# Ophiase/Stochastic-Vector-Oracle-Consensus

Hardware: AMD Instinct MI355X
Metric: consensus updates/sec (N oracles x D dims, batched) (higher is better)
Workload: dtype fp32; 1 GPU; model=svoc-consensus N=256 D=4096 streaming (f=32, constrained), global_batch=1024, seq_len=4096, parallelism=dp1, engine_mode=fast, storage=fp32, n_oracles=256, dimension=4096, n_failing=32, hip_graph=True, backend_world=1, stream_pool=89, independent_failing=False, transactional=False, fast_transactional=True, pipeline_chunks=2

## Files before the change

csrc/bindings/torch_ops.cpp:

```cpp
#include <cstdlib>
#include <ATen/ATen.h>
#include <c10/hip/HIPStream.h>
#include <torch/library.h>

#include <thread>

#include "../engine/engine.hpp"
#include "svoc/route.hpp"
#include "svoc/ops.hpp"

namespace svoc {
namespace {

int cpu_threads() {
  static int n = [] {
    unsigned h = std::thread::hardware_concurrency();
    return (int)(h == 0 ? 1 : (h > 32 ? 32 : h));
  }();
  return n;
}

void check_out(const at::Tensor& t, at::ScalarType dt, std::initializer_list<int64_t> shape, const char* name,
               const at::Device& dev) {
  TORCH_CHECK(t.scalar_type() == dt, name, ": wrong dtype ", t.scalar_type());
// ... 26 lines not shown
  check_out(qr, at::kFloat, {B, N}, "qr", dev);
  check_out(reliable, at::kByte, {B, N}, "reliable", dev);
  check_out(status, at::kInt, {B}, "status", dev);
}

void fast_round_cpu(const at::Tensor& values, const c10::optional<at::Tensor>& active, int64_t D,
                    int64_t n_failing, bool constrained, double max_spread, at::Tensor c1, at::Tensor cons,
                    at::Tensor skew, at::Tensor kurt, at::Tensor rel, at::Tensor qr, at::Tensor reliable,
                    at::Tensor status, int64_t wave_hint, int64_t mode, int64_t rel_dim, bool legacy,
                    const c10::optional<at::Tensor>& work, const c10::optional<at::Tensor>& stats,
                    const c10::optional<at::Tensor>& upd_rows, const c10::optional<at::Tensor>& upd_oracle,
                    const c10::optional<at::Tensor>& upd_status, int64_t upd_per_inst,
                    const c10::optional<at::Tensor>& rst_saved, const c10::optional<at::Tensor>& rst_saved_en,
                    const c10::optional<at::Tensor>& rst_enabled, const c10::optional<at::Tensor>& rst_n_active,
                    const c10::optional<at::Tensor>& pend_rows, const c10::optional<at::Tensor>& pend_oracle,
                    const c10::optional<at::Tensor>& pend_status) {
  (void)wave_hint;
  (void)work;
  (void)stats;
  TORCH_CHECK(!upd_rows.has_value() || !upd_rows->defined(), "fused transactional streaming is a GPU path");
  TORCH_CHECK(!rst_saved.has_value() || !rst_saved->defined(), "in-kernel rollback is a GPU path");
  TORCH_CHECK(!pend_rows.has_value() || !pend_rows->defined(), "the deferred commit is a GPU path");
  (void)pend_oracle;
  (void)pend_status;
  (void)rst_saved_en;
  (void)rst_enabled;
  (void)rst_n_active;
  (void)upd_oracle;
  (void)upd_status;
  (void)upd_per_inst;
  fast_round_checks(values, D, c1, cons, skew, kurt, rel, qr, reliable, status);
  const int64_t B = values.size(0), N = values.size(1), ld = values.size(2), is = values.stride(0);
// ... 33 lines not shown
  fb.rel_dim = rel_dim;
  fb.legacy = legacy;
  fast_round_batch_cpu(fb, cpu_threads());
}

void fast_round_hip(const at::Tensor& values, const c10::optional<at::Tensor>& active, int64_t D,
                    int64_t n_failing, bool constrained, double max_spread, at::Tensor c1, at::Tensor cons,
                    at::Tensor skew, at::Tensor kurt, at::Tensor rel, at::Tensor qr, at::Tensor reliable,
                    at::Tensor status, int64_t wave_hint, int64_t mode, int64_t rel_dim, bool legacy,
                    const c10::optional<at::Tensor>& work, const c10::optional<at::Tensor>& stats,
                    const c10::optional<at::Tensor>& upd_rows, const c10::optional<at::Tensor>& upd_oracle,
                    const c10::optional<at::Tensor>& upd_status, int64_t upd_per_inst,
                    const c10::optional<at::Tensor>& rst_saved, const c10::optional<at::Tensor>& rst_saved_en,
                    const c10::optional<at::Tensor>& rst_enabled, const c10::optional<at::Tensor>& rst_n_active,
                    const c10::optional<at::Tensor>& pend_rows, const c10::optional<at::Tensor>& pend_oracle,
                    const c10::optional<at::Tensor>& pend_status) {
  fast_round_checks(values, D, c1, cons, skew, kurt, rel, qr, reliable, status);
  TORCH_CHECK(values.scalar_type() == at::kBFloat16 || values.scalar_type() == at::kFloat,
              "GPU fast path stores values in bf16 or fp32");
  const bool f32 = values.scalar_type() == at::kFloat;
  const int64_t B = values.size(0), N = values.size(1), ld = values.size(2);
  if (f32) {
    TORCH_CHECK(N >= 2 && N <= 4096, "GPU fp32 fast path supports 2 <= N <= 4096 oracles");
    TORCH_CHECK(B < (1ll << 31) && D < (1 << 30), "size limits");
    TORCH_CHECK(N * ld * 4 < (1ll << 31) && fast_work_words(D) * 4 < (1ll << 31),
                "instance too large for 32-bit buffer offsets (N * ld * 4 B and the workspace must stay < 2 GiB)");
  }
  if (!f32) {
    TORCH_CHECK(N >= 2 && N <= 4096, "GPU fast path supports 2 <= N <= 4096 oracles");
    TORCH_CHECK(ld % 8 == 0, "row stride (ld) must be a multiple of 8 bf16 (16 B)");
    TORCH_CHECK(((uintptr_t)values.data_ptr() & 15) == 0 && values.stride(0) % 8 == 0, "values must be 16-B aligned");
// ... 40 lines not shown
    p.work = (uint32_t*)wtmp.data_ptr();
    p.work_fresh = 1;
  }
  {
    const char* wc = std::getenv("SVOC_WIN_CANCEL");
    p.win_cancel = wc ? (float)std::atof(wc) : 64.f;
  }
  p.work_pairs = (int)fast_work_pairs(D);
  p.work_stride = words;
  auto stream = c10::hip::getCurrentHIPStream(values.device().index()).stream();
  p.c1_out = mode == 0 ? c1.data_ptr<float>() : nullptr;
  if (stats.has_value() && stats->defined()) {
    TORCH_CHECK(stats->scalar_type() == at::kInt && stats->numel() >= 1 && stats->device() == values.device(),
                "stats: int32 [>= 1] on the values' device ([0] += pruned-network fallbacks)");
    p.net_fallbacks = (unsigned int*)stats->data_ptr();
  }
  for (const c10::optional<at::Tensor>* t : {&upd_rows, &upd_oracle, &upd_status, &rst_saved, &rst_saved_en,
                                              &rst_enabled, &rst_n_active})
    TORCH_CHECK(!t->has_value() || !(*t)->defined() || (*t)->device() == values.device(),
                "fast_round: every update / rollback tensor must be on the values' device");
  if (upd_rows.has_value() && upd_rows->defined()) {
    TORCH_CHECK(upd_per_inst <= route.fused_max_u, "fused streaming: this round's kernel takes at most ",
                route.fused_max_u, " updates per instance (fp32 storage, whole constrained rounds on the window "
                "kernel; svoc.ops.fast_route)");
    TORCH_CHECK(upd_per_inst > 0 && upd_oracle.has_value() && upd_status.has_value(), "fused streaming: "
                "upd_oracle, upd_status and upd_per_inst > 0 go with upd_rows");
    const int64_t n = B * upd_per_inst;
    TORCH_CHECK(upd_rows->scalar_type() == values.scalar_type() && upd_rows->is_contiguous() && upd_rows->dim() == 2 &&
                    upd_rows->size(0) == n && upd_rows->size(1) == D && upd_rows->device() == values.device(),
                "upd_rows: contiguous [B * U, D] in the values' dtype on the values' device");
// ... 293 lines not shown
  const int rc = svoc_exact_verdict(&p, stream);
  TORCH_CHECK(rc == 0, "svoc_exact_verdict launch failed: ", rc);
}

}
}

TORCH_LIBRARY(svoc, m) {
  m.def(
      "fast_round(Tensor values, Tensor? active, int D, int n_failing, bool constrained, float max_spread, "
      "Tensor(a!) c1, Tensor(b!) consensus, Tensor(c!) skew, Tensor(d!) kurt, Tensor(e!) rel, Tensor(f!) qr, "
      "Tensor(g!) reliable, Tensor(h!) status, int wave_hint=0, int mode=0, int rel_dim=0, bool legacy=False, "
      "Tensor? work=None, Tensor(i!)? stats=None, Tensor? upd_rows=None, Tensor? upd_oracle=None, "
      "Tensor(j!)? upd_status=None, int upd_per_inst=0, Tensor? rst_saved=None, Tensor? rst_saved_en=None, "
      "Tensor(k!)? rst_enabled=None, Tensor(l!)? rst_n_active=None, Tensor? pend_rows=None, "
      "Tensor? pend_oracle=None, Tensor? pend_status=None) -> ()");
  m.def(
      "exact_round(Tensor values, Tensor? active, int n_failing, bool constrained, int max_spread, "
      "Tensor(a!) c1, Tensor(b!) consensus, Tensor(c!) skew, Tensor(d!) kurt, Tensor(e!) rel, Tensor(f!) qr, "
      "Tensor(g!) reliable, Tensor(h!) status, bool legacy=False, int mode=0, int rel_dim=0, "
      "Tensor(i!)? stats=None) -> ()");
  m.def(
      "exact_verdict(Tensor values, Tensor? active, int n_failing, bool constrained, int max_spread, "
      "Tensor(a!) rel, Tensor(b!) status, bool legacy, Tensor(c!)? stats=None, Tensor(d!)? vstats=None) -> ()");
  m.def("fast_route(int storage, int N, int D, int ld, int n_failing, bool constrained, bool legacy, int mode, "
        "int wave_hint, int work) -> int[]", &svoc::fast_route_op);
  m.def("exact_route(int N, int D, int elem_bytes, int n_failing, bool constrained, bool legacy, int mode) -> int[]",
        &svoc::exact_route_op);
  m.def("fast_work_words(int D) -> int", [](int64_t D) { return svoc::fast_work_words(D); });
  m.def("fast_win_h(int N, int n_failing) -> int",
        [](int64_t N, int64_t f) { return (int64_t)svoc::fast_win_h((int)N, (int)f); });
  svoc::register_extra_defs(m);
}

TORCH_LIBRARY_IMPL(svoc, CPU, m) {
  m.impl("fast_round", &svoc::fast_round_cpu);
  m.impl("exact_round", &svoc::exact_round_cpu);
  m.impl("exact_verdict", &svoc::exact_verdict_cpu);
  svoc::register_extra_cpu(m);
}

TORCH_LIBRARY_IMPL(svoc, CUDA, m) {
  m.impl("fast_round", &svoc::fast_round_hip);
  m.impl("exact_round", &svoc::exact_round_hip);
  m.impl("exact_verdict", &svoc::exact_verdict_hip);
  svoc::register_extra_hip(m);
// ... 2 lines not shown
```

csrc/include/svoc/launch.hpp:

```cpp
#pragma once

#include <stdint.h>

namespace svoc {

struct FastParams {
  const void* values;
  const uint8_t* active;
  int64_t inst_stride;
  int B, N, D, ld;
  int n_failing;
  int constrained;
  float max_spread;
  int wave_hint;
  int mode;
  int rel_dim;
  float* c1;
  float* consensus;
  float* skew;
  float* kurt;
  float* rel;
  float* qr;
  uint8_t* reliable;
  int32_t* status;
// ... 7 lines not shown
  unsigned int* net_fallbacks;
  const float* upd_rows;
  const int64_t* upd_oracle;
  int32_t* upd_status;
  int upd_per_inst;
  const float* pend_rows;
  const int64_t* pend_oracle;
  const int32_t* pend_status;
  const void* rst_saved;
  const uint8_t* rst_saved_en;
  const int64_t* rst_oracle;
  int32_t* rst_status;
  uint8_t* rst_enabled;
  int32_t* rst_n_active;
  int rst_U;
};

inline int64_t fast_work_pairs(int64_t D) { return ((D + 1) / 2 + 255) / 256 * 256; }
inline int64_t fast_work_stage_word(int64_t D) { return fast_work_pairs(D) * (2 * 17 + 8 + 2); }
constexpr int kWinfStageCols = 2 * 17 + 4 + 1;
inline int64_t fast_work_words(int64_t D) { return fast_work_pairs(D) * 2 * (kWinfStageCols + 3); }
inline int64_t fast_work_numel(int64_t B, int64_t D) { return B * fast_work_words(D); }

inline int fast_win_h(int N, int f) {
  const int R = N - f, a = N / 2 - R / 2;
  if (a + 1 <= 5 && f - a + 1 <= 5) return 5;
  if (a + 1 <= 17 && f - a + 1 <= 17) return 17;
  return 0;
}

struct LestParams {
// ... 104 lines not shown
```

csrc/kernels/consensus_fast_winf.hip:

```cpp
#include <hip/hip_runtime.h>
#include <stdint.h>

#include <type_traits>
#include <utility>

#include "svoc/bufload.hpp"
#include "svoc/route.hpp"
#include "svoc/slabdma.hpp"
#include "svoc/rankmask.hpp"
#include "svoc/sortnet.hpp"
#include "svoc/status.hpp"
#include "svoc/verdict.hpp"

namespace svoc {

template <bool CONS>
SVOC_DEV uint32_t fkey(uint32_t raw) {
  if constexpr (CONS) return raw ^ 0x80000000u;
  else return f32_key(raw);
}
template <bool CONS>
SVOC_DEV float fkey_val(uint32_t k) {
  if constexpr (CONS) return __builtin_bit_cast(float, k ^ 0x80000000u);
  else return key_f32(k);
// ... 85 lines not shown
SVOC_DEV bool try_pruned(uint32_t (&r)[64], int seg, int lane, uint32_t (&w)[WN], uint32_t& lo, uint32_t& hi,
                         uint32_t& e0, uint32_t& e63) {
  if constexpr (WN == H && H == 17) {
    bool ok;
    sort_oem<64>(r);
    e0 = r[0];
    e63 = r[63];
    window_group_pruned_sorted<P, H>(r, seg, lane, w, lo, hi, ok);
    return ok;
  } else {
    return false;
  }
}


template <int NSEG, int WAVES, int H, bool CONS, int MODE, bool FUSED = false, bool DEFER = false, bool WIDE = false>
__global__ __launch_bounds__(WAVES * 64) __attribute__((amdgpu_waves_per_eu(2))) void consensus_fast_winf_kernel(FastParams p) {
#pragma clang fp contract(off)
  constexpr int P = 64 / NSEG;
  constexpr int NPAD = 64 * NSEG;
  constexpr int W = WAVES * P;
  constexpr int NT = WAVES * 64;
  constexpr int KEEP = 64 / P;
  constexpr bool PASS1 = MODE != 2;
  __shared__ __attribute__((aligned(16))) uint32_t slab[PASS1 ? WAVES * 64 * 64 : 1];
  __shared__ __attribute__((aligned(16))) float qr_part[WAVES * NPAD];
  __shared__ float qr_lds[NPAD];
  __shared__ uint64_t relmask[4];
  __shared__ int urow[32];
  __shared__ float misc_f[2];
  __shared__ int misc_i[3];
  __shared__ uint32_t redo[128];
  __shared__ int smap[FUSED ? NPAD : 1];
  __shared__ int spend[DEFER ? NPAD : 1];
  __shared__ uint32_t badu[8];

  const int b = blockIdx.x;
  static_assert(!FUSED || (MODE == 0 && CONS), "fused streaming: whole constrained rounds");
  static_assert(!DEFER || FUSED, "deferred commit: a mode of the fused path");
  static_assert(!WIDE || (FUSED && !DEFER), "9-bit piece map: the fused path at 256 updates per instance");
  constexpr bool fused = FUSED;
  const int U = fused ? p.upd_per_inst : 0;
  if (p.active && !p.active[b]) {
    for (int t = threadIdx.x; t < U; t += WAVES * 64) p.upd_status[(int64_t)b * U + t] = ST_NOT_ACTIVE;
    return;
  }
  const int tid = threadIdx.x, lane = tid & 63, wave = __builtin_amdgcn_readfirstlane(tid >> 6);
  if (tid < 32) urow[tid] = 0;
  if (tid == 0) misc_i[2] = 0;
  if (tid < 128) redo[tid] = 0u;
  const int seg = lane / P, cw = lane % P;
  const int N = p.N, D = p.D;
  const int rowb = p.ld * 4;
  const float* inst = (const float*)p.values + (int64_t)b * p.inst_stride;
  const __amdgpu_buffer_rsrc_t rs = instance_rsrc(inst, (uint32_t)(N * rowb));
  const BufDesc rsd = buf_desc(inst, (uint32_t)(N * rowb));
  const int nslab = (D + W - 1) / W;
  const int Dc = 2 * p.work_pairs;
  const __amdgpu_buffer_rsrc_t ws = instance_rsrc(p.work + (int64_t)b * p.work_stride, (uint32_t)(p.work_stride * 4));
  const int MOM = 2 * H * Dc * 4;
  const int LST = MOM + 4 * Dc * 4;
  const int STG = Dc * kWinfStageCols * 4;
  const float* urows = fused ? p.upd_rows + (int64_t)b * U * D : inst;
  const uint32_t ubytes = fused ? (uint32_t)(U * D * 4) : 0u;
  const __amdgpu_buffer_rsrc_t rb = instance_rsrc(urows, ubytes);
// ... 118 lines not shown
            rsd, rbd, reg_o, rowb_o, s * W + wave * P,
            [&](int k) { return ((pm[k / 4] >> (8 * (k % 4))) & 0xffu) | (((ph >> k) & 1u) << 8); },
            [&](int, uint32_t fb) { return (int)__umul24(fb, (unsigned)d4) + cbm; });
      } else
      dma.issue_mapped(
          rsd, rbd, reg_o, rowb_o, s * W + wave * P,
          [&](int k) { return (pm[k / 4] >> (8 * (k % 4))) & 0xffu; },
          [&](int, uint32_t fb) { return (int)__umul24(fb, (unsigned)d4) + cbm; });
    } else {
      dma.issue(rsd, region, rowb, s * W + wave * P);
    }
  };
  for (int attempt = 0; attempt < 2; ++attempt) {
  if (fused) map_pieces();
  if (pass1_slabs > 0) issue_slab(0);
  auto slab_body = [&](auto full_c, int s) __attribute__((always_inline)) {
    constexpr bool FULL = decltype(full_c)::value;
    const int col = s * W + wave * P + cw;
    const bool vc = FULL || col < D;
    int nvl = nv, nll = nl;
    asm volatile("" : "+v"(nvl), "+v"(nll));
    float c1v;
    const uint32_t mW = vc ? 0xffffffffu : 0u;
    RawRows xs;
    __builtin_amdgcn_s_waitcnt(0x0F70);
    if constexpr (DEFER) {
      if (attempt == 0) {
        uint32_t pm[4] = {pmap[0], pmap[1], pmap[2], pmap[3]};
        asm volatile("" : "+v"(pm[0]), "+v"(pm[1]), "+v"(pm[2]), "+v"(pm[3]));
        int rowb_o = rowb;
        asm volatile("" : "+s"(rowb_o));
        const int c0 = s * W + wave * P;
// ... 80 lines not shown
            window_group<NSEG, P, H>(r, seg, lane, wk, klo, khi);
          }
        };
        pruned_net(full_c);
        if constexpr (NSEG == 1) {
#pragma unroll
          for (int m = 0; m < H; ++m) {
            bstore(ws, wk[m], col * 4, 2 * m * Dc * 4);
            bstore(ws, wk[H + m], (Dc + col) * 4, 2 * m * Dc * 4);
          }
        } else {
          constexpr int slo = NSEG == 2 ? 0 : 1;
          if (seg == slo || seg == slo + 1) {
            const int part = seg - slo;
#pragma unroll
            for (int m = 0; m < H; ++m) bstore(ws, wk[m], (part * Dc + col) * 4, 2 * m * Dc * 4);
          }
        }
      } else {
        median_group<NSEG>(r, klo, khi);
      }
      c1v = 0.5f * (fkey_val<CONS>(klo) + fkey_val<CONS>(khi));
    }
    if (seg == 0 && vc) p.c1[(int64_t)b * D + col] = c1v;
    const float cq = vc ? c1v : 0.f;
    f32x2 s1 = {0.f, 0.f}, s2 = s1, s3 = s1, s4 = s1;
    if constexpr (ACC64) {
      qr_moments_regs<!FULL, !FULL>(xs, nvl, cq, mW, acc, s1, s2, s3, s4);
    } else {
      f32x2 slab_acc[32];
#pragma unroll
// ... 5 lines not shown
    if constexpr (NSEG == 4) {
      t1 += xor_lane<16>(t1); t2 += xor_lane<16>(t2); t3 += xor_lane<16>(t3); t4 += xor_lane<16>(t4);
    }
    if constexpr (NSEG >= 2) {
      t1 += xor_lane<32>(t1); t2 += xor_lane<32>(t2); t3 += xor_lane<32>(t3); t4 += xor_lane<32>(t4);
    }
    if (seg == 0) {
      bstore(ws, f2u(t1), col * 4, MOM);
      bstore(ws, f2u(t2), col * 4, MOM + Dc * 4);
      bstore(ws, f2u(t3), col * 4, MOM + 2 * Dc * 4);
      bstore(ws, f2u(t4), col * 4, MOM + 3 * Dc * 4);
    }
  };
  if constexpr (PASS1) {
    const int nfull = N == NPAD ? min(D / W, pass1_slabs) : 0;
#pragma nounroll
    for (int s = 0; s < nfull; ++s) slab_body(std::true_type{}, s);
#pragma nounroll
    for (int s = nfull; s < pass1_slabs; ++s) slab_body(std::false_type{}, s);
  }
  if (!fused) break;
  __syncthreads();
  uint32_t anybad = 0u;
#pragma unroll
  for (int w = 0; w < 8; ++w) anybad |= badu[w];
  if (anybad == 0u || attempt == 1) break;
  if constexpr (FUSED) {
    for (int t = tid; t < NPAD; t += NT)
      if (smap[t] >= 0 && bad_slot(smap[t])) smap[t] = -1;
  }
  __syncthreads();
#pragma unroll
  for (int i = 0; i < (ACC64 ? 32 : 1); ++i) acc[i] = f32x2{0.f, 0.f};
#pragma unroll
// ... 49 lines not shown
      misc_f[1] = v.rel2;
      misc_i[0] = v.status;
      misc_i[1] = 0;
    }
  }
  __syncthreads();
  if (misc_i[0] != ST_OK) {
    if (tid == 0) p.status[b] = misc_i[0];
    upd_out(misc_i[0]);
    return;
  }

  if (CONS && !p.legacy) {
    const bool inwin = f + H <= N / 2;
    const int fr = first_reliable_row<4>(relmask);
    bool zv = false;
#pragma nounroll
    for (int base = wave * 64; base < D; base += WAVES * 64) {
      const int col = base + lane;
      const int pc = col < D ? col : D - 1;
      bool cand = col < D;
      if (inwin) {
        const uint32_t lo = bload(ws, pc * 4, 0), hi = ~bload(ws, (Dc + pc) * 4, 0);
        cand = cand && fkey_val<true>(lo) == fkey_val<true>(hi);
      }
      if (__ballot(cand)) {
        const float r0 = u2f(row_load(fr, pc * 4));
        for (int i = fr + 1; i < N; ++i) {
          if (!((relmask[i >> 6] >> (i & 63)) & 1)) continue;
          cand = cand && u2f(row_load(i, pc * 4)) == r0;
        }
        zv = zv || cand;
      }
    }
    if (zv) misc_i[1] = 1;
    __syncthreads();
    if (misc_i[1]) {
      if (tid == 0) p.status[b] = ST_ZERO_VARIANCE;
// ... 9 lines not shown
  }

  const double n = (double)R;
  const MomKd mk = mom_kd(n);
  const int sh = H - 1 - (N / 2 - R / 2);
  const int64_t ob = (int64_t)b * D;
  bool zv = false;
  constexpr int NS = CONS ? 2 * H : 32;
  constexpr int NW = CONS ? H : 1;
  struct PBWords {
    uint32_t uw[NS];
    uint32_t wl[NW], wu[NW];
    uint32_t am[4];
    float c1c;
  };
  auto pb_load = [&](int base, PBWords& q) __attribute__((always_inline)) {
    const int col = base + lane;
    const int pc = col < D ? col : D - 1;
    const int vo = pc * 4;
    int shl = sh, fl = f;
    asm volatile("" : "+s"(shl), "+s"(fl));
    const int s0 = CONS ? shl : 0;
    const uint64_t realm = ((fl >= 64 ? ~0ull : (1ull << fl) - 1)) << s0;
    q.c1c = p.c1[ob + pc];
#pragma unroll
    for (int t = 0; t < NS; ++t) {
      const int row = t - s0;
      const bool real = (realm >> t) & 1;
      q.uw[t] = 0u;
      if (CONS || real) q.uw[t] = row_load(__builtin_amdgcn_readfirstlane(urow[real ? row : 0]), vo);
    }
    if constexpr (CONS) {
#pragma unroll
      for (int m = 0; m < H; ++m) {
        q.wl[m] = bload(ws, pc * 4, 2 * m * Dc * 4);
        q.wu[m] = ~bload(ws, (Dc + pc) * 4, 2 * m * Dc * 4);
      }
    }
#pragma unroll
    for (int k = 0; k < 4; ++k) q.am[k] = bload(ws, pc * 4, MOM + k * Dc * 4);
  };
  float* const o_lds = reinterpret_cast<float*>(slab);
  const bool ldso = CONS && PASS1 && D <= 4096;
  auto pb_col = [&](auto ldso_c, int base, const PBWords& cur) __attribute__((always_inline)) {
    constexpr bool LDSO = decltype(ldso_c)::value;
    const int col = base + lane;
    const float c1c = cur.c1c;
    int shl = sh, fl = f;
    asm volatile("" : "+s"(shl), "+s"(fl));
    const int s0 = CONS ? shl : 0;
    const uint64_t realm = ((fl >= 64 ? ~0ull : (1ull << fl) - 1)) << s0;
    const uint64_t lowm = (1ull << s0) - 1;
    float u1 = 0.f, u2 = 0.f, u3 = 0.f, u4 = 0.f;
#pragma unroll
    for (int t = 0; t < NS; ++t) {
      if ((realm >> t) & 1) {
        const float y = u2f(cur.uw[t]) - c1c;
        const float q = y * y;
        u1 += y;
        u2 += q;
        u3 = __builtin_fmaf(q, y, u3);
        u4 = __builtin_fmaf(q, q, u4);
      }
    }
    float cons_v = 0.f;
    if constexpr (CONS) {
      auto cands = [&](const auto& z) __attribute__((always_inline)) {
        uint32_t clo = ~0u, chi = ~0u;
#pragma unroll
        for (int m = 0; m < H; ++m) {
          const uint32_t wl = cur.wl[m], wu = cur.wu[m];
          clo = kmin(clo, winf_cand(wl, z(m)));
          if (m) chi = kmin(chi, winf_cand(wl, z(m - 1)));
          clo = kmin(clo, winf_cand(wu, z(2 * H - 1 - m)));
          chi = kmin(chi, winf_cand(wu, z(2 * H - 2 - m)));
        }
        cons_v = 0.5f * (fkey_val<true>(clo) + fkey_val<true>(chi));
      };
      constexpr int NF = H == 17 ? 32 : 8;
      if (s0 == 0 && fl == NF) {
        uint32_t z[NF];
#pragma unroll
        for (int t = 0; t < NF; ++t) z[t] = cur.uw[t] ^ 0x80000000u;
        sort_oem<NF>(z);
        cands([&](int t) __attribute__((always_inline)) { return t < NF ? z[t < NF ? t : 0] : ~0u; });
      } else {
        uint32_t z[64];
#pragma unroll
        for (int t = 0; t < 64; ++t) {
          if (t < 2 * H) {
            const uint32_t mreal = 0u - (uint32_t)((realm >> t) & 1);
            const uint32_t kx = (0x80000000u & mreal) | (~mreal & (0u - (uint32_t)(((~lowm) >> t) & 1)));
            z[t] = (cur.uw[t] & mreal) ^ kx;
          } else {
            z[t] = ~0u;
          }
        }
        sort_oem<64>(z);
        cands([&](int t) __attribute__((always_inline)) { return z[t]; });
      }
    }
    const double a1 = (double)u2f(cur.am[0]), a2 = (double)u2f(cur.am[1]);
    const double a3 = (double)u2f(cur.am[2]), a4 = (double)u2f(cur.am[3]);
    const double r1 = a1 - (double)u1, r2 = a2 - (double)u2, r3 = a3 - (double)u3, r4 = a4 - (double)u4;
    if (col < D) {
      const double rdl = r1 * mk.in, rmu2 = r2 * mk.in - rdl * rdl;
      const double wc = (double)p.win_cancel;
      const bool good = r2 > 0.0 && a2 <= wc * r2 && a4 <= wc * r4 && rdl * rdl <= 4.0 * rmu2;
      if constexpr (LDSO) {
        o_lds[col] = cons_v;
        o_lds[3 * D + col] = c1c;
      } else if (CONS) {
        p.consensus[ob + col] = cons_v;
        if (MODE == 0 && p.c1_out) p.c1_out[ob + col] = c1c;
      }
      if (good) {
        double dl;
        float sk, ku;
        const bool nz = moments_from_sums_d(mk, r1, r2, r3, r4, dl, sk, ku);
        if constexpr (LDSO) {
          o_lds[D + col] = p.legacy ? 0.f : sk;
          o_lds[2 * D + col] = p.legacy ? 0.f : ku;
        } else if (CONS) {
          p.skew[ob + col] = p.legacy ? 0.f : sk;
          p.kurt[ob + col] = p.legacy ? 0.f : ku;
        } else {
          stage_out(ws, STG, Dc, 0, col, (float)((double)c1c + dl));
          stage_out(ws, STG, Dc, 1, col, p.legacy ? 0.f : sk);
          stage_out(ws, STG, Dc, 2, col, p.legacy ? 0.f : ku);
          zv |= !nz;
        }
      } else if constexpr (LDSO) {
        atomicOr(&redo[col >> 5], 1u << (col & 31));
      } else {
        const int k = atomicAdd(&misc_i[2], 1);
        bstore(ws, (uint32_t)col, k * 4, LST);
      }
    }
  };
  if (ldso) {
    __builtin_amdgcn_s_waitcnt(0x0F70);
    PBWords cur;
    pb_load(wave * 64, cur);
#pragma nounroll
    for (int base = wave * 64; base < D; base += WAVES * 64) {
      PBWords nxt;
      if (base + WAVES * 64 < D) pb_load(base + WAVES * 64, nxt);
      asm volatile("" ::: "memory");
      pb_col(std::true_type{}, base, cur);
      cur = nxt;
    }
  } else {
#pragma nounroll
    for (int base = wave * 64; base < D; base += WAVES * 64) {
      PBWords cur;
      pb_load(base, cur);
      pb_col(std::false_type{}, base, cur);
    }
  }
  if (!CONS && zv && !p.legacy) misc_i[1] = 1;
  __syncthreads();
  auto cleanup_col = [&](int col) __attribute__((always_inline)) {
      const float cc = p.c1[ob + col];
      const float* xc = inst + col;
      float y[NSEG];
      float t1 = 0.f;
#pragma unroll
      for (int g = 0; g < NSEG; ++g) {
        const int i = g * 64 + lane;
        const bool use = i < N && ((relmask[g] >> lane) & 1);
        float xv = 0.f;
        if (use) {
          int u = -1, q = -1;
          if constexpr (FUSED) u = smap[i];
          if constexpr (DEFER) q = spend[i];
          xv = u >= 0 ? urows[(int64_t)u * D + col] : q >= 0 ? prows[(int64_t)q * D + col] : xc[(int64_t)i * p.ld];
        }
        y[g] = use ? xv - cc : 0.f;
        t1 += y[g];
      }
      t1 += xor_lane<1>(t1); t1 += xor_lane<2>(t1); t1 += xor_lane<4>(t1);
      t1 += xor_lane<8>(t1); t1 += xor_lane<16>(t1); t1 += xor_lane<32>(t1);
      const float mu = t1 / (float)R;
      float c1s = 0.f, t2 = 0.f, t3 = 0.f, t4 = 0.f;
#pragma unroll
      for (int g = 0; g < NSEG; ++g) {
        const int i = g * 64 + lane;
        const bool use = i < N && ((relmask[g] >> lane) & 1);
        const float d = use ? y[g] - mu : 0.f;
        const float q = d * d;
        c1s += d;
        t2 += q;
        t3 = fmaf(q, d, t3);
        t4 = fmaf(q, q, t4);
// ... 13 lines not shown
          o_lds[2 * D + col] = p.legacy ? 0.f : ku;
        } else if (CONS) {
          p.skew[ob + col] = p.legacy ? 0.f : sk;
          p.kurt[ob + col] = p.legacy ? 0.f : ku;
        } else {
          stage_out(ws, STG, Dc, 0, col, (float)((double)cc + (double)mu + dl));
          stage_out(ws, STG, Dc, 1, col, p.legacy ? 0.f : sk);
          stage_out(ws, STG, Dc, 2, col, p.legacy ? 0.f : ku);
          if (!nz && !p.legacy) misc_i[1] = 1;
        }
      }
  };
  if (ldso) {
    int k = 0;
    for (int w32 = 0; w32 < (D + 31) / 32; ++w32) {
      uint32_t bits = redo[w32];
      while (bits) {
        const int c = __builtin_ctz(bits);
        bits &= bits - 1;
        if (k % WAVES == wave) cleanup_col(w32 * 32 + c);
        ++k;
      }
    }
    __syncthreads();
    const bool c1o = MODE == 0 && p.c1_out;
    if ((D & 3) == 0) {
      for (int i = tid; i < D / 4; i += NT) {
        const float4* o4 = reinterpret_cast<const float4*>(o_lds);
        reinterpret_cast<float4*>(p.consensus + ob)[i] = o4[i];
        reinterpret_cast<float4*>(p.skew + ob)[i] = o4[D / 4 + i];
        reinterpret_cast<float4*>(p.kurt + ob)[i] = o4[2 * (D / 4) + i];
        if (c1o) reinterpret_cast<float4*>(p.c1_out + ob)[i] = o4[3 * (D / 4) + i];
      }
    } else {
      for (int i = tid; i < D; i += NT) {
        p.consensus[ob + i] = o_lds[i];
        p.skew[ob + i] = o_lds[D + i];
        p.kurt[ob + i] = o_lds[2 * D + i];
        if (c1o) p.c1_out[ob + i] = o_lds[3 * D + i];
      }
    }
  } else {
    const int nredo = misc_i[2];
    if (nredo) {
      for (int k = wave; k < nredo; k += WAVES) {
        cleanup_col((int)__builtin_amdgcn_readfirstlane(__builtin_amdgcn_raw_buffer_load_b32(ws, 0, LST + k * 4, 1)));
      }
      __syncthreads();
    }
  }
  if (!CONS) {
    if (misc_i[1]) {
      if (tid == 0) p.status[b] = ST_ZERO_VARIANCE;
      return;
    }
    commit_staged<NT>(ws, STG, Dc, D, tid, p.consensus + ob, p.skew + ob, p.kurt + ob);
    if (MODE == 0 && p.c1_out)
      for (int c = tid; c < D; c += NT) p.c1_out[ob + c] = p.c1[ob + c];
    for (int t = tid; t < N; t += NT) {
      p.reliable[(int64_t)b * N + t] = (relmask[t >> 6] >> (t & 63)) & 1;
      p.qr[(int64_t)b * N + t] = qr_lds[t];
    }
  }
  if (tid == 0) {
    p.rel[2 * (int64_t)b] = misc_f[0];
    p.rel[2 * (int64_t)b + 1] = misc_f[1];
    p.status[b] = ST_OK;
  }
  upd_out(ST_OK);
}

template <int NSEG, int WAVES, int H, bool CONS>
static void launch_winf_w(const FastParams& p, hipStream_t stream) {
  if constexpr (CONS) {
    if (p.upd_rows && p.pend_rows) {
      hipLaunchKernelGGL((consensus_fast_winf_kernel<NSEG, WAVES, H, CONS, 0, true, true>), dim3(p.B),
                         dim3(WAVES * 64), 0, stream, p);
      return;
    }
    if (p.upd_rows && p.upd_per_inst > 255) {
      hipLaunchKernelGGL((consensus_fast_winf_kernel<NSEG, WAVES, H, CONS, 0, true, false, true>), dim3(p.B),
                         dim3(WAVES * 64), 0, stream, p);
      return;
    }
    if (p.upd_rows) {
      hipLaunchKernelGGL((consensus_fast_winf_kernel<NSEG, WAVES, H, CONS, 0, true>), dim3(p.B), dim3(WAVES * 64), 0,
                         stream, p);
      return;
    }
  }
  if (p.mode == 1) hipLaunchKernelGGL((consensus_fast_winf_kernel<NSEG, WAVES, H, CONS, 1>), dim3(p.B), dim3(WAVES * 64), 0, stream, p);
  else if (p.mode == 2) hipLaunchKernelGGL((consensus_fast_winf_kernel<NSEG, WAVES, H, CONS, 2>), dim3(p.B), dim3(WAVES * 64), 0, stream, p);
  else hipLaunchKernelGGL((consensus_fast_winf_kernel<NSEG, WAVES, H, CONS, 0>), dim3(p.B), dim3(WAVES * 64), 0, stream, p);
}

template <int NSEG, int H, bool CONS>
static void launch_winf_c(const FastParams& p, hipStream_t stream) {
  launch_winf_w<NSEG, 4, H, CONS>(p, stream);
}

template <int NSEG>
static void launch_winf(const FastParams& p, int H, hipStream_t stream) {
  if (!p.constrained) launch_winf_c<NSEG, 5, false>(p, stream);
  else if (H == 5) launch_winf_c<NSEG, 5, true>(p, stream);
  else launch_winf_c<NSEG, 17, true>(p, stream);
}

}
// ... 22 lines not shown
```

svoc/engine.py:

```python
from __future__ import annotations

import os
from typing import Dict, Optional, Sequence

import numpy as np
import torch

from . import estimators
from . import ops as svops
from .config import WSAD, ConsensusConfig
from .status import Status


def _round_up(x: int, m: int) -> int:
    return (x + m - 1) // m * m


class _PendingBatches:

    FOLD_AT = 8

    def __init__(self, eng: "ConsensusEngine"):
        self.e = eng
        self.entries = []
# ... 101 lines not shown
        self._winner = torch.full((B, N), -1, dtype=torch.int32, device=dev)
        self._active = torch.zeros(B, dtype=torch.uint8, device=dev)
        self.wave_hint = 0
        self.rounds = 0
        self.failing_mask: Optional[torch.Tensor] = None
        self._lest = None
        self._lest_route = None
        self._lest_explicit = rank_weights is not None
        if lest_rows is not None:
            self._lest = estimators.pack(*lest_rows[0]).to(dev)
            self._lest_route = lest_rows[1]
        self._work = None
        self._routes: Dict[int, tuple] = {}
        self._xroute = None
        self.transactional = mode == "fast"
        self._net_fb = torch.zeros(1, dtype=torch.int32, device=dev) if (mode == "fast" and dev.type == "cuda") else None
        self._xstats = torch.zeros(2, dtype=torch.int32, device=dev) if (mode == "exact" and dev.type == "cuda") else None
        self._vstats = torch.zeros(3, dtype=torch.int32, device=dev) if (mode == "exact" and dev.type == "cuda") else None
        self._pending = _PendingBatches(self)
        self._save_bufs: Dict[tuple, tuple] = {}
        self._all_active = False
        self._pipe_streams = None
        self._pipe_open = False
        self._pipe_held = None
        self._defer = None
        self._last_st = None
        self._dshard_pending = None
        self._dshard_pending_rows = None
        self._dshard_ctx = None
        self._dshard_shadow = None
        self.metrics_fx = torch.zeros(4, dtype=torch.int64, device=dev)
# ... 140 lines not shown
            if w is not None and sl is not None:
                words = w.numel() // self.B
                w = w[sl.start * words:sl.stop * words]
            if self._lest is not None:
                if batch:
                    raise RuntimeError("the rank-weighted round takes no update / rollback batch")
                self._ops.lest_round(v(self.values), active, self.D, self.cfg.n_failing_oracles, self.cfg.constrained,
                                     float(self.cfg.unconstrained_max_spread), self._lest, v(self.c1),
                                     v(self.consensus), v(self.skew), v(self.kurt), v(self.rel), v(self.qr),
                                     v(self.reliable), v(self.status), w)
            else:
                self._ops.fast_round(v(self.values), active, self.D, self.cfg.n_failing_oracles,
                                     self.cfg.constrained, float(self.cfg.unconstrained_max_spread), v(self.c1),
                                     v(self.consensus), v(self.skew), v(self.kurt), v(self.rel), v(self.qr),
                                     v(self.reliable), v(self.status), self.wave_hint, 0, 0, self.cfg.legacy, w,
                                     self._net_fb, **batch)
        else:
            self._ops.exact_round(v(self.values), active, self.cfg.n_failing_oracles, self.cfg.constrained,
                                  self.cfg.max_spread_wsad, v(self.c1), v(self.consensus), v(self.skew), v(self.kurt),
                                  v(self.rel), v(self.qr), v(self.reliable), v(self.status), self.cfg.legacy,
                                  stats=self._xstats)
        if then is not None:
            then()
        self._track_update(slice(None) if sl is None else sl)
        self._ops.round_epilogue(active, v(self.status), v(self.rel), v(self.consensus_active), v(self.touched),
                                 self.metrics_fx)

    def run_round(self, only_touched: bool = True) -> None:
        self.pipeline_join()
        self._round_over(None, only_touched, then=self._restore_pending if self.mode == "fast" else None)
        self.rounds += 1
# ... 175 lines not shown
            self._pipe_held = None

    def work(self) -> Optional[torch.Tensor]:
        if not self._gpu_fast():
            return None
        if not (self._lest_route if self._lest is not None else self._route()).needs_work:
            return None
        if self._work is None:
            self._work = torch.empty(svops.fast_work_numel(self.B, self.D), dtype=torch.int32,
                                     device=self.device)
        return self._work

    def net_stats(self) -> Dict[str, int]:
        self.pipeline_join()
        if self._net_fb is None or self._lest is not None or not self._route().pruned:
            return {"slab_networks": 0, "fallbacks": 0}
        processed = int(self.metrics_fx[2].item())
        return {"slab_networks": processed * (self.D // 64) * 4, "fallbacks": int(self._net_fb.item())}

    def exact_routing(self) -> Dict[str, int]:
        self.pipeline_join()
        processed = int(self.metrics_fx[2].item())
        if self._xstats is None:
            return {"processed": processed, "wide_column": 0, "i128": 0}
        x = self._xstats.tolist()
        return {"processed": processed, "wide_column": int(x[0]), "i128": int(x[1])}

    def verdict_routing(self) -> Dict[str, int]:
        self.pipeline_join()
        if self._vstats is None:
            return {"verdict": 0, "fallback": 0, "mismatch": 0}
        v = self._vstats.tolist()
        return {"verdict": int(v[0]), "fallback": int(v[1]), "mismatch": int(v[2])}
# ... 148 lines not shown

    def randomize(self, seed: int = 0, a: float = 20.0, failing_low: float = 0.0) -> None:
        self.pipeline_join()
        from .models.oracle_gen import beta_failing_oracles
        g = torch.Generator(device=self.device).manual_seed(seed)
        x, self.failing_mask = beta_failing_oracles(self.B, self.N, self.D, self.cfg.n_failing_oracles, a, g,
                                                    self.device, return_mask=True)
        if self.mode == "exact":
            self.values[:, :, : self.D] = (x.double() * WSAD).to(torch.int64).to(self.vdtype)
        else:
            self.values[:, :, : self.D] = x.to(self.vdtype)
        self.enabled.fill_(1)
        self.n_active.fill_(self.N)
        self.touched.fill_(1)
        self._all_active = True

    def get_consensus_value(self, i: Optional[int] = None) -> torch.Tensor:
        self.pipeline_join()
        return self.consensus if i is None else self.consensus[i]

    def get_first_pass_consensus_reliability(self, i: Optional[int] = None):
        self.pipeline_join()
        return self.rel[:, 0] if i is None else self.rel[i, 0]

    def get_second_pass_consensus_reliability(self, i: Optional[int] = None):
        self.pipeline_join()
        return self.rel[:, 1] if i is None else self.rel[i, 1]

    def get_skewness(self, i: Optional[int] = None):
        self.pipeline_join()
# ... 20 lines not shown
```

svoc/ops/__init__.py:

```python
from __future__ import annotations

import os
import threading
from typing import NamedTuple

import torch

_LIB = os.path.join(os.path.dirname(os.path.dirname(os.path.abspath(__file__))), "_C.so")
_lock = threading.Lock()
_loaded = False


class NativeExtensionMissing(RuntimeError):
    pass


def load(build_if_missing: bool = False) -> None:
    global _loaded
    if _loaded:
        return
    with _lock:
        if _loaded:
            return
        if not os.path.exists(_LIB):
# ... 71 lines not shown
def lest_route(storage: str, N: int, D: int, ld: int, n_failing: int, constrained: bool, legacy: bool = False,
               mode: int = 0) -> LestRoute:
    return LestRoute(*ops().lest_route(STORAGE[storage], N, D, ld, n_failing, bool(constrained), bool(legacy), mode))


def fast_work_words(D: int) -> int:
    return ops().fast_work_words(D)


def fast_work_numel(B: int, D: int) -> int:
    return B * fast_work_words(D)


def fast_win_h(N: int, f: int) -> int:
    return ops().fast_win_h(N, f)
```

Measured before the change: 616,000 consensus rounds/s.

## Add adaptive narrow-window path for constrained winf kernel with per-column fallback

Adds a per-instance hint so that, once the previous round shows the window rarely fails, the winf kernel only stores and reloads the inner HS of the H window slices. It also skips loading the extra sorted-network rows on the fast path. Columns where the narrowed window cannot be trusted are flagged and recomputed in cleanup by an exact rank-based median over the reliable oracles. The hint is updated on device each round, and counters are added to the stats tensor. The aim is to cut workspace stores and loads and compare work, at the cost of a costlier cleanup per fallback column plus extra LDS and atomics.

```diff
diff --git a/csrc/bindings/torch_ops.cpp b/csrc/bindings/torch_ops.cpp
--- a/csrc/bindings/torch_ops.cpp
+++ b/csrc/bindings/torch_ops.cpp
@@ -64,8 +64,9 @@
                     const c10::optional<at::Tensor>& rst_saved, const c10::optional<at::Tensor>& rst_saved_en,
                     const c10::optional<at::Tensor>& rst_enabled, const c10::optional<at::Tensor>& rst_n_active,
                     const c10::optional<at::Tensor>& pend_rows, const c10::optional<at::Tensor>& pend_oracle,
-                    const c10::optional<at::Tensor>& pend_status) {
+                    const c10::optional<at::Tensor>& pend_status, const c10::optional<at::Tensor>& win_hint) {
   (void)wave_hint;
+  (void)win_hint;
   (void)work;
   (void)stats;
   TORCH_CHECK(!upd_rows.has_value() || !upd_rows->defined(), "fused transactional streaming is a GPU path");
@@ -129,7 +130,7 @@
                     const c10::optional<at::Tensor>& rst_saved, const c10::optional<at::Tensor>& rst_saved_en,
                     const c10::optional<at::Tensor>& rst_enabled, const c10::optional<at::Tensor>& rst_n_active,
                     const c10::optional<at::Tensor>& pend_rows, const c10::optional<at::Tensor>& pend_oracle,
-                    const c10::optional<at::Tensor>& pend_status) {
+                    const c10::optional<at::Tensor>& pend_status, const c10::optional<at::Tensor>& win_hint) {
   fast_round_checks(values, D, c1, cons, skew, kurt, rel, qr, reliable, status);
   TORCH_CHECK(values.scalar_type() == at::kBFloat16 || values.scalar_type() == at::kFloat,
               "GPU fast path stores values in bf16 or fp32");
@@ -200,6 +201,14 @@
     TORCH_CHECK(stats->scalar_type() == at::kInt && stats->numel() >= 1 && stats->device() == values.device(),
                 "stats: int32 [>= 1] on the values' device ([0] += pruned-network fallbacks)");
     p.net_fallbacks = (unsigned int*)stats->data_ptr();
+    if (stats->numel() >= 3) p.win_stats = (unsigned int*)stats->data_ptr() + 1;
+  }
+  if (win_hint.has_value() && win_hint->defined()) {
+    TORCH_CHECK(win_hint->scalar_type() == at::kInt && win_hint->is_contiguous() && win_hint->numel() == B &&
+                    win_hint->device() == values.device(),
+                "win_hint: contiguous int32 [B] on the values' device");
+    const char* wn = std::getenv("SVOC_WIN_NARROW");
+    if (f32 && mode == 0 && !(wn && wn[0] == '0')) p.win_hint = win_hint->data_ptr<int32_t>();
   }
   for (const c10::optional<at::Tensor>* t : {&upd_rows, &upd_oracle, &upd_status, &rst_saved, &rst_saved_en,
                                               &rst_enabled, &rst_n_active})
@@ -523,7 +532,7 @@
       "Tensor? work=None, Tensor(i!)? stats=None, Tensor? upd_rows=None, Tensor? upd_oracle=None, "
       "Tensor(j!)? upd_status=None, int upd_per_inst=0, Tensor? rst_saved=None, Tensor? rst_saved_en=None, "
       "Tensor(k!)? rst_enabled=None, Tensor(l!)? rst_n_active=None, Tensor? pend_rows=None, "
-      "Tensor? pend_oracle=None, Tensor? pend_status=None) -> ()");
+      "Tensor? pend_oracle=None, Tensor? pend_status=None, Tensor(m!)? win_hint=None) -> ()");
   m.def(
       "exact_round(Tensor values, Tensor? active, int n_failing, bool constrained, int max_spread, "
       "Tensor(a!) c1, Tensor(b!) consensus, Tensor(c!) skew, Tensor(d!) kurt, Tensor(e!) rel, Tensor(f!) qr, "
@@ -539,6 +548,7 @@
   m.def("fast_work_words(int D) -> int", [](int64_t D) { return svoc::fast_work_words(D); });
   m.def("fast_win_h(int N, int n_failing) -> int",
         [](int64_t N, int64_t f) { return (int64_t)svoc::fast_win_h((int)N, (int)f); });
+  m.def("fast_win_narrow_hs() -> int", []() { return (int64_t)svoc::kWinfNarrowHs; });
   svoc::register_extra_defs(m);
 }
 
diff --git a/csrc/include/svoc/launch.hpp b/csrc/include/svoc/launch.hpp
--- a/csrc/include/svoc/launch.hpp
+++ b/csrc/include/svoc/launch.hpp
@@ -45,7 +45,13 @@
   uint8_t* rst_enabled;
   int32_t* rst_n_active;
   int rst_U;
+  int32_t* win_hint;
+  unsigned int* win_stats;
 };
+#ifndef SVOC_WINF_HS
+#define SVOC_WINF_HS 11
+#endif
+constexpr int kWinfNarrowHs = SVOC_WINF_HS;
 
 inline int64_t fast_work_pairs(int64_t D) { return ((D + 1) / 2 + 255) / 256 * 256; }
 inline int64_t fast_work_stage_word(int64_t D) { return fast_work_pairs(D) * (2 * 17 + 8 + 2); }
diff --git a/csrc/kernels/consensus_fast_winf.hip b/csrc/kernels/consensus_fast_winf.hip
--- a/csrc/kernels/consensus_fast_winf.hip
+++ b/csrc/kernels/consensus_fast_winf.hip
@@ -123,7 +123,8 @@
 }
 
 
-template <int NSEG, int WAVES, int H, bool CONS, int MODE, bool FUSED = false, bool DEFER = false, bool WIDE = false>
+template <int NSEG, int WAVES, int H, bool CONS, int MODE, bool FUSED = false, bool DEFER = false, bool WIDE = false,
+          bool NARROW = false>
 __global__ __launch_bounds__(WAVES * 64) __attribute__((amdgpu_waves_per_eu(2))) void consensus_fast_winf_kernel(FastParams p) {
 #pragma clang fp contract(off)
   constexpr int P = 64 / NSEG;
@@ -143,6 +144,12 @@
   __shared__ int smap[FUSED ? NPAD : 1];
   __shared__ int spend[DEFER ? NPAD : 1];
   __shared__ uint32_t badu[8];
+  __shared__ uint32_t redow[NARROW ? 128 : 1];
+  __shared__ int win_fail[1];
+  static_assert(!NARROW || (NSEG == 4 && H == 17 && CONS && MODE == 0), "narrow window: N = 256, whole constrained rounds");
+  constexpr int HS = NARROW ? kWinfNarrowHs : H;
+  constexpr int KN = H - HS;
+  static_assert(HS >= 1 && (!NARROW || KN >= 1), "narrow window: 1 <= HS < H");
 
   const int b = blockIdx.x;
   static_assert(!FUSED || (MODE == 0 && CONS), "fused streaming: whole constrained rounds");
@@ -158,6 +165,12 @@
   if (tid < 32) urow[tid] = 0;
   if (tid == 0) misc_i[2] = 0;
   if (tid < 128) redo[tid] = 0u;
+  bool nar = false;
+  if constexpr (NARROW) {
+    nar = __builtin_amdgcn_readfirstlane(p.win_hint[b]) != 0 && p.D <= 4096;
+    if (tid < 128) redow[tid] = 0u;
+    if (tid == 0) win_fail[0] = 0;
+  }
   const int seg = lane / P, cw = lane % P;
   const int N = p.N, D = p.D;
   const int rowb = p.ld * 4;
@@ -306,8 +319,9 @@
   for (int attempt = 0; attempt < 2; ++attempt) {
   if (fused) map_pieces();
   if (pass1_slabs > 0) issue_slab(0);
-  auto slab_body = [&](auto full_c, int s) __attribute__((always_inline)) {
+  auto slab_body = [&](auto full_c, auto nar_c, int s) __attribute__((always_inline)) {
     constexpr bool FULL = decltype(full_c)::value;
+    constexpr int M0 = decltype(nar_c)::value ? KN : 0;
     const int col = s * W + wave * P + cw;
     const bool vc = FULL || col < D;
     int nvl = nv, nll = nl;
@@ -418,7 +432,7 @@
           if (seg == slo || seg == slo + 1) {
             const int part = seg - slo;
 #pragma unroll
-            for (int m = 0; m < H; ++m) bstore(ws, wk[m], (part * Dc + col) * 4, 2 * m * Dc * 4);
+            for (int m = M0; m < H; ++m) bstore(ws, wk[m], (part * Dc + col) * 4, 2 * m * Dc * 4);
           }
         }
       } else {
@@ -454,10 +468,15 @@
   };
   if constexpr (PASS1) {
     const int nfull = N == NPAD ? min(D / W, pass1_slabs) : 0;
+    if (NARROW && nar) {
 #pragma nounroll
-    for (int s = 0; s < nfull; ++s) slab_body(std::true_type{}, s);
+      for (int s = 0; s < nfull; ++s) slab_body(std::true_type{}, std::integral_constant<bool, NARROW>{}, s);
+    } else {
 #pragma nounroll
-    for (int s = nfull; s < pass1_slabs; ++s) slab_body(std::false_type{}, s);
+      for (int s = 0; s < nfull; ++s) slab_body(std::true_type{}, std::false_type{}, s);
+    }
+#pragma nounroll
+    for (int s = nfull; s < pass1_slabs; ++s) slab_body(std::false_type{}, std::false_type{}, s);
   }
   if (!fused) break;
   __syncthreads();
@@ -537,6 +556,7 @@
   if (CONS && !p.legacy) {
     const bool inwin = f + H <= N / 2;
     const int fr = first_reliable_row<4>(relmask);
+    const int zp = nar ? 2 * KN * Dc * 4 : 0;
     bool zv = false;
 #pragma nounroll
     for (int base = wave * 64; base < D; base += WAVES * 64) {
@@ -544,7 +564,7 @@
       const int pc = col < D ? col : D - 1;
       bool cand = col < D;
       if (inwin) {
-        const uint32_t lo = bload(ws, pc * 4, 0), hi = ~bload(ws, (Dc + pc) * 4, 0);
+        const uint32_t lo = bload(ws, pc * 4, zp), hi = ~bload(ws, (Dc + pc) * 4, zp);
         cand = cand && fkey_val<true>(lo) == fkey_val<true>(hi);
       }
       if (__ballot(cand)) {
@@ -584,7 +604,11 @@
     uint32_t am[4];
     float c1c;
   };
-  auto pb_load = [&](int base, PBWords& q) __attribute__((always_inline)) {
+  constexpr int NF = H == 17 ? 32 : 8;
+  int win_failed = 0;
+  auto pb_load = [&](auto nar_c, int base, PBWords& q) __attribute__((always_inline)) {
+    constexpr bool NAR = decltype(nar_c)::value;
+    constexpr int M0 = NAR ? KN : 0;
     const int col = base + lane;
     const int pc = col < D ? col : D - 1;
     const int vo = pc * 4;
@@ -593,16 +617,18 @@
     const int s0 = CONS ? shl : 0;
     const uint64_t realm = ((fl >= 64 ? ~0ull : (1ull << fl) - 1)) << s0;
     q.c1c = p.c1[ob + pc];
+    const bool sfree = NAR && s0 == 0 && fl == NF;
 #pragma unroll
     for (int t = 0; t < NS; ++t) {
       const int row = t - s0;
       const bool real = (realm >> t) & 1;
       q.uw[t] = 0u;
-      if (CONS || real) q.uw[t] = row_load(__builtin_amdgcn_readfirstlane(urow[real ? row : 0]), vo);
+      if ((CONS || real) && !(NAR && t >= NF && sfree))
+        q.uw[t] = row_load(__builtin_amdgcn_readfirstlane(urow[real ? row : 0]), vo);
     }
     if constexpr (CONS) {
 #pragma unroll
-      for (int m = 0; m < H; ++m) {
+      for (int m = M0; m < H; ++m) {
         q.wl[m] = bload(ws, pc * 4, 2 * m * Dc * 4);
         q.wu[m] = ~bload(ws, (Dc + pc) * 4, 2 * m * Dc * 4);
       }
@@ -612,8 +638,10 @@
   };
   float* const o_lds = reinterpret_cast<float*>(slab);
   const bool ldso = CONS && PASS1 && D <= 4096;
-  auto pb_col = [&](auto ldso_c, int base, const PBWords& cur) __attribute__((always_inline)) {
+  auto pb_col = [&](auto ldso_c, auto nar_c, int base, const PBWords& cur) __attribute__((always_inline)) {
     constexpr bool LDSO = decltype(ldso_c)::value;
+    constexpr bool NAR = decltype(nar_c)::value;
+    constexpr int M0 = NAR ? KN : 0;
     const int col = base + lane;
     const float c1c = cur.c1c;
     int shl = sh, fl = f;
@@ -634,11 +662,12 @@
       }
     }
     float cons_v = 0.f;
+    bool wtrust = true;
     if constexpr (CONS) {
       auto cands = [&](const auto& z) __attribute__((always_inline)) {
         uint32_t clo = ~0u, chi = ~0u;
 #pragma unroll
-        for (int m = 0; m < H; ++m) {
+        for (int m = M0; m < H; ++m) {
           const uint32_t wl = cur.wl[m], wu = cur.wu[m];
           clo = kmin(clo, winf_cand(wl, z(m)));
           if (m) chi = kmin(chi, winf_cand(wl, z(m - 1)));
@@ -646,8 +675,10 @@
           chi = kmin(chi, winf_cand(wu, z(2 * H - 2 - m)));
         }
         cons_v = 0.5f * (fkey_val<true>(clo) + fkey_val<true>(chi));
+        if constexpr (NARROW) {
+          wtrust = z(KN - 1) < cur.wl[KN] && z(2 * H - 2 - KN) > cur.wu[KN];
+        }
       };
-      constexpr int NF = H == 17 ? 32 : 8;
       if (s0 == 0 && fl == NF) {
         uint32_t z[NF];
 #pragma unroll
@@ -677,6 +708,9 @@
       const double rdl = r1 * mk.in, rmu2 = r2 * mk.in - rdl * rdl;
       const double wc = (double)p.win_cancel;
       const bool good = r2 > 0.0 && a2 <= wc * r2 && a4 <= wc * r4 && rdl * rdl <= 4.0 * rmu2;
+      if constexpr (NAR) {
+        if (!wtrust) atomicOr(&redow[col >> 5], 1u << (col & 31));
+      }
       if constexpr (LDSO) {
         o_lds[col] = cons_v;
         o_lds[3 * D + col] = c1c;
@@ -707,34 +741,43 @@
         bstore(ws, (uint32_t)col, k * 4, LST);
       }
     }
+    if constexpr (NARROW) win_failed += __popcll(__ballot(col < D && !wtrust));
   };
   if (ldso) {
     __builtin_amdgcn_s_waitcnt(0x0F70);
-    PBWords cur;
-    pb_load(wave * 64, cur);
+    auto pb_loop = [&](auto nar_c) __attribute__((always_inline)) {
+      PBWords cur;
+      pb_load(nar_c, wave * 64, cur);
 #pragma nounroll
-    for (int base = wave * 64; base < D; base += WAVES * 64) {
-      PBWords nxt;
-      if (base + WAVES * 64 < D) pb_load(base + WAVES * 64, nxt);
-      asm volatile("" ::: "memory");
-      pb_col(std::true_type{}, base, cur);
-      cur = nxt;
-    }
+      for (int base = wave * 64; base < D; base += WAVES * 64) {
+        PBWords nxt;
+        if (base + WAVES * 64 < D) pb_load(nar_c, base + WAVES * 64, nxt);
+        asm volatile("" ::: "memory");
+        pb_col(std::true_type{}, nar_c, base, cur);
+        cur = nxt;
+      }
+    };
+    if (NARROW && nar) pb_loop(std::integral_constant<bool, NARROW>{});
+    else pb_loop(std::false_type{});
   } else {
 #pragma nounroll
     for (int base = wave * 64; base < D; base += WAVES * 64) {
       PBWords cur;
-      pb_load(base, cur);
-      pb_col(std::false_type{}, base, cur);
-    }
+      pb_load(std::false_type{}, base, cur);
+      pb_col(std::false_type{}, std::false_type{}, base, cur);
+    }
+  }
+  if constexpr (NARROW) {
+    if (lane == 0 && win_failed) atomicAdd(&win_fail[0], win_failed);
   }
   if (!CONS && zv && !p.legacy) misc_i[1] = 1;
   __syncthreads();
-  auto cleanup_col = [&](int col) __attribute__((always_inline)) {
+  auto cleanup_col = [&](int col, bool mom, bool win) __attribute__((always_inline)) {
       const float cc = p.c1[ob + col];
       const float* xc = inst + col;
       float y[NSEG];
       float t1 = 0.f;
+      uint32_t ck[NSEG];
 #pragma unroll
       for (int g = 0; g < NSEG; ++g) {
         const int i = g * 64 + lane;
@@ -748,6 +791,44 @@
         }
         y[g] = use ? xv - cc : 0.f;
         t1 += y[g];
+        ck[g] = fkey<true>(f2u(xv));
+      }
+      if constexpr (NARROW) {
+        if (win) {
+          int lt[NSEG], le[NSEG];
+#pragma unroll
+          for (int g = 0; g < NSEG; ++g) lt[g] = le[g] = 0;
+#pragma unroll
+          for (int h = 0; h < NSEG; ++h) {
+            const uint64_t rm = relmask[h];
+#pragma nounroll
+            for (int j = 0; j < 64; ++j) {
+              if (!((rm >> j) & 1)) continue;
+              const uint32_t kk = (uint32_t)__builtin_amdgcn_readlane((int)ck[h], j);
+#pragma unroll
+              for (int g = 0; g < NSEG; ++g) {
+                lt[g] += kk < ck[g];
+                le[g] += kk <= ck[g];
+              }
+            }
+          }
+          const int rl = R / 2 - 1, rh = R / 2;
+          uint32_t klo = 0u, khi = 0u;
+#pragma unroll
+          for (int g = 0; g < NSEG; ++g) {
+            const bool use = g * 64 + lane < N && ((relmask[g] >> lane) & 1);
+            if (use && lt[g] <= rl && rl < le[g]) klo = ck[g];
+            if (use && lt[g] <= rh && rh < le[g]) khi = ck[g];
+          }
+          klo = kmax(klo, xor_lane_u32<1>(klo)); khi = kmax(khi, xor_lane_u32<1>(khi));
+          klo = kmax(klo, xor_lane_u32<2>(klo)); khi = kmax(khi, xor_lane_u32<2>(khi));
+          klo = kmax(klo, xor_lane_u32<4>(klo)); khi = kmax(khi, xor_lane_u32<4>(khi));
+          klo = kmax(klo, xor_lane_u32<8>(klo)); khi = kmax(khi, xor_lane_u32<8>(khi));
+          klo = kmax(klo, xor_lane_u32<16>(klo)); khi = kmax(khi, xor_lane_u32<16>(khi));
+          klo = kmax(klo, xor_lane_u32<32>(klo)); khi = kmax(khi, xor_lane_u32<32>(khi));
+          if (lane == 0) o_lds[col] = 0.5f * (fkey_val<true>(klo) + fkey_val<true>(khi));
+        }
+        if (!mom) return;
       }
       t1 += xor_lane<1>(t1); t1 += xor_lane<2>(t1); t1 += xor_lane<4>(t1);
       t1 += xor_lane<8>(t1); t1 += xor_lane<16>(t1); t1 += xor_lane<32>(t1);
@@ -791,11 +872,14 @@
   if (ldso) {
     int k = 0;
     for (int w32 = 0; w32 < (D + 31) / 32; ++w32) {
-      uint32_t bits = redo[w32];
+      const uint32_t bm = redo[w32];
+      uint32_t bw = 0u;
+      if constexpr (NARROW) bw = redow[w32];
+      uint32_t bits = bm | bw;
       while (bits) {
         const int c = __builtin_ctz(bits);
         bits &= bits - 1;
-        if (k % WAVES == wave) cleanup_col(w32 * 32 + c);
+        if (k % WAVES == wave) cleanup_col(w32 * 32 + c, (bm >> c) & 1, (bw >> c) & 1);
         ++k;
       }
     }
@@ -821,7 +905,8 @@
     const int nredo = misc_i[2];
     if (nredo) {
       for (int k = wave; k < nredo; k += WAVES) {
-        cleanup_col((int)__builtin_amdgcn_readfirstlane(__builtin_amdgcn_raw_buffer_load_b32(ws, 0, LST + k * 4, 1)));
+        cleanup_col((int)__builtin_amdgcn_readfirstlane(__builtin_amdgcn_raw_buffer_load_b32(ws, 0, LST + k * 4, 1)), true,
+                    false);
       }
       __syncthreads();
     }
@@ -843,32 +928,50 @@
     p.rel[2 * (int64_t)b] = misc_f[0];
     p.rel[2 * (int64_t)b + 1] = misc_f[1];
     p.status[b] = ST_OK;
+    if constexpr (NARROW) {
+      const int nf = win_fail[0];
+      p.win_hint[b] = nf <= D / 64 && D <= 4096 ? 1 : 0;
+      if (nar && p.win_stats) {
+        atomicAdd(p.win_stats, 1u);
+        if (nf) atomicAdd(p.win_stats + 1, (unsigned)nf);
+      }
+    }
   }
   upd_out(ST_OK);
+}
+
+template <int NSEG, int WAVES, int H, bool CONS, int MODE, bool FUSED, bool DEFER, bool WIDE>
+static void launch_winf_k(const FastParams& p, hipStream_t stream) {
+  if constexpr (NSEG == 4 && H == 17 && CONS && MODE == 0) {
+    if (p.win_hint) {
+      auto k = consensus_fast_winf_kernel<NSEG, WAVES, H, CONS, MODE, FUSED, DEFER, WIDE, true>;
+      hipLaunchKernelGGL(k, dim3(p.B), dim3(WAVES * 64), 0, stream, p);
+      return;
+    }
+  }
+  auto k = consensus_fast_winf_kernel<NSEG, WAVES, H, CONS, MODE, FUSED, DEFER, WIDE>;
+  hipLaunchKernelGGL(k, dim3(p.B), dim3(WAVES * 64), 0, stream, p);
 }
 
 template <int NSEG, int WAVES, int H, bool CONS>
 static void launch_winf_w(const FastParams& p, hipStream_t stream) {
   if constexpr (CONS) {
     if (p.upd_rows && p.pend_rows) {
-      hipLaunchKernelGGL((consensus_fast_winf_kernel<NSEG, WAVES, H, CONS, 0, true, true>), dim3(p.B),
-                         dim3(WAVES * 64), 0, stream, p);
+      launch_winf_k<NSEG, WAVES, H, CONS, 0, true, true, false>(p, stream);
       return;
     }
     if (p.upd_rows && p.upd_per_inst > 255) {
-      hipLaunchKernelGGL((consensus_fast_winf_kernel<NSEG, WAVES, H, CONS, 0, true, false, true>), dim3(p.B),
-                         dim3(WAVES * 64), 0, stream, p);
+      launch_winf_k<NSEG, WAVES, H, CONS, 0, true, false, true>(p, stream);
       return;
     }
     if (p.upd_rows) {
-      hipLaunchKernelGGL((consensus_fast_winf_kernel<NSEG, WAVES, H, CONS, 0, true>), dim3(p.B), dim3(WAVES * 64), 0,
-                         stream, p);
+      launch_winf_k<NSEG, WAVES, H, CONS, 0, true, false, false>(p, stream);
       return;
     }
   }
-  if (p.mode == 1) hipLaunchKernelGGL((consensus_fast_winf_kernel<NSEG, WAVES, H, CONS, 1>), dim3(p.B), dim3(WAVES * 64), 0, stream, p);
-  else if (p.mode == 2) hipLaunchKernelGGL((consensus_fast_winf_kernel<NSEG, WAVES, H, CONS, 2>), dim3(p.B), dim3(WAVES * 64), 0, stream, p);
-  else hipLaunchKernelGGL((consensus_fast_winf_kernel<NSEG, WAVES, H, CONS, 0>), dim3(p.B), dim3(WAVES * 64), 0, stream, p);
+  if (p.mode == 1) launch_winf_k<NSEG, WAVES, H, CONS, 1, false, false, false>(p, stream);
+  else if (p.mode == 2) launch_winf_k<NSEG, WAVES, H, CONS, 2, false, false, false>(p, stream);
+  else launch_winf_k<NSEG, WAVES, H, CONS, 0, false, false, false>(p, stream);
 }
 
 template <int NSEG, int H, bool CONS>
diff --git a/svoc/engine.py b/svoc/engine.py
--- a/svoc/engine.py
+++ b/svoc/engine.py
@@ -139,7 +139,9 @@
         self._routes: Dict[int, tuple] = {}
         self._xroute = None
         self.transactional = mode == "fast"
-        self._net_fb = torch.zeros(1, dtype=torch.int32, device=dev) if (mode == "fast" and dev.type == "cuda") else None
+        self._net_fb = torch.zeros(3, dtype=torch.int32, device=dev) if (mode == "fast" and dev.type == "cuda") else None
+        self._win_hint = (torch.zeros(B, dtype=torch.int32, device=dev)
+                          if (mode == "fast" and dev.type == "cuda" and self.vdtype == torch.float32) else None)
         self._xstats = torch.zeros(2, dtype=torch.int32, device=dev) if (mode == "exact" and dev.type == "cuda") else None
         self._vstats = torch.zeros(3, dtype=torch.int32, device=dev) if (mode == "exact" and dev.type == "cuda") else None
         self._pending = _PendingBatches(self)
@@ -310,7 +312,8 @@
                                      self.cfg.constrained, float(self.cfg.unconstrained_max_spread), v(self.c1),
                                      v(self.consensus), v(self.skew), v(self.kurt), v(self.rel), v(self.qr),
                                      v(self.reliable), v(self.status), self.wave_hint, 0, 0, self.cfg.legacy, w,
-                                     self._net_fb, **batch)
+                                     self._net_fb, win_hint=None if self._win_hint is None else v(self._win_hint),
+                                     **batch)
         else:
             self._ops.exact_round(v(self.values), active, self.cfg.n_failing_oracles, self.cfg.constrained,
                                   self.cfg.max_spread_wsad, v(self.c1), v(self.consensus), v(self.skew), v(self.kurt),
@@ -516,9 +519,11 @@
     def net_stats(self) -> Dict[str, int]:
         self.pipeline_join()
         if self._net_fb is None or self._lest is not None or not self._route().pruned:
-            return {"slab_networks": 0, "fallbacks": 0}
+            return {"slab_networks": 0, "fallbacks": 0, "narrow_rounds": 0, "narrow_fallback_cols": 0}
         processed = int(self.metrics_fx[2].item())
-        return {"slab_networks": processed * (self.D // 64) * 4, "fallbacks": int(self._net_fb.item())}
+        fb = self._net_fb.tolist()
+        return {"slab_networks": processed * (self.D // 64) * 4, "fallbacks": int(fb[0]), "narrow_rounds": int(fb[1]),
+                "narrow_fallback_cols": int(fb[2])}
 
     def exact_routing(self) -> Dict[str, int]:
         self.pipeline_join()
@@ -697,6 +702,8 @@
         self.n_active.fill_(self.N)
         self.touched.fill_(1)
         self._all_active = True
+        if self._win_hint is not None:
+            self._win_hint.zero_()
 
     def get_consensus_value(self, i: Optional[int] = None) -> torch.Tensor:
         self.pipeline_join()
diff --git a/svoc/ops/__init__.py b/svoc/ops/__init__.py
--- a/svoc/ops/__init__.py
+++ b/svoc/ops/__init__.py
@@ -109,3 +109,7 @@
 
 def fast_win_h(N: int, f: int) -> int:
     return ops().fast_win_h(N, f)
+
+
+def fast_win_narrow_hs() -> int:
+    return ops().fast_win_narrow_hs()
```

After: 639,000 consensus rounds/s, median of 6. 1.04x the previous value.
